# quantum-bitss/Audio-Backdoor-Attack

Hardware: AMD Instinct MI355X
Metric: poisoned+clean utterances/sec/GPU; ASR & clean-acc parity vs reference (higher is better)
Workload: dtype f32 (conv GEMMs as exact 3-way bf16 splits, 6 MFMA terms, fp32 accumulate)

## Files before the change

### audio-backdoor-attack_amd/_lib.py

```python
from __future__ import annotations

import ctypes as C
import os
import threading

HERE = os.path.dirname(os.path.abspath(__file__))
LIB_PATH = os.environ.get("ABD_LIB", os.path.join(HERE, "libabd.so"))

ABD_MEL_HTK, ABD_MEL_SLANEY = 0, 1
ABD_PAD_REFLECT, ABD_PAD_CONSTANT = 0, 1
INJECT_NONE, INJECT_ADD, INJECT_SNR_WINDOW, INJECT_HALF_MIX, INJECT_DEPLOY, INJECT_DEPLOY_CLAMP = 0, 1, 2, 3, 4, 5
MFCC_INFO = {"fast": 0, "ppb": 1, "chunks": 2, "mel_path": 3, "dct_kernel": 4, "bwd_ok": 5}
MFCC_MEL_PATHS = ("generic", "half_slot", "segmented", "blue_slots")
MFCC_DCT_KERNELS = ("plain", "lds", "mfma1", "mfma2", "mfma3")
METRICS_WORDS = 8

EXPORTS = (
    "abd_last_error", "abd_version",
    "abd_mfcc_plan_create", "abd_mfcc_plan_destroy", "abd_mfcc_plan_frames", "abd_mfcc_plan_describe",
    "abd_mfcc_plan_info",
    "abd_mfcc_workspace_bytes", "abd_mfcc_f32", "abd_mfcc_rows_f32", "abd_gather_rows_f32", "abd_inject_waveform_f32", "abd_inject_workspace_bytes",
    "abd_inject_row_scales",
    "abd_pydub_overlay_i16", "abd_mfcc_deploy_backward_workspace_bytes", "abd_mfcc_deploy_backward",
    "abd_smallcnn_create", "abd_smallcnn_destroy", "abd_smallcnn_param_count", "abd_smallcnn_param_offsets",
    "abd_smallcnn_flat_features", "abd_smallcnn_workspace_bytes", "abd_smallcnn_workspace_offset", "abd_smallcnn_bn1_folded", "abd_smallcnn_conv2_planes",
    "abd_smallcnn_train_step",
    "abd_smallcnn_apply", "abd_smallcnn_forward", "abd_smallcnn_backward", "abd_smallcnn_eval", "abd_adam_f32",
    "abd_smallcnn_input_grad_workspace_bytes", "abd_smallcnn_input_grad",
    "abd_smallcnn_ablate_workspace_bytes", "abd_smallcnn_ablate_eval",
    "abd_segment_norms_workspace_bytes", "abd_segment_norms_f32", "abd_perturb_f32", "abd_sgd_f32",
    "abd_smallcnn_finetune_reg_workspace_bytes", "abd_smallcnn_finetune_reg_step",
    "abd_row_abs_sums_f32", "abd_smallcnn_unlearn_workspace_bytes", "abd_smallcnn_unlearn_step",
    "abd_reinit_weights_f32", "abd_smallcnn_unlearn_run", "abd_nwc_pair_f32",
    "abd_smallcnn_hidden_sums", "abd_smallcnn_fcprune_workspace_bytes", "abd_smallcnn_fcprune_eval",
    "abd_smallcnn_pruned_finetune_workspace_bytes", "abd_smallcnn_pruned_finetune_step",
    "abd_lstmattn_create", "abd_lstmattn_destroy", "abd_lstmattn_param_count", "abd_lstmattn_param_offsets",
    "abd_lstmattn_tile_rows", "abd_lstmattn_workspace_bytes", "abd_lstmattn_workspace_offset", "abd_lstmattn_forward",
    "abd_lstmattn_backward", "abd_lstmattn_train_step", "abd_lstmattn_eval",
    "abd_per_utterance_lstmattn_workspace_bytes", "abd_per_utterance_lstmattn_forward",
    "abd_rnn_create", "abd_rnn_destroy", "abd_rnn_param_count", "abd_rnn_param_offsets", "abd_rnn_tile_info",
    "abd_rnn_workspace_bytes", "abd_rnn_workspace_offset", "abd_rnn_forward", "abd_rnn_backward",
    "abd_rnn_train_step", "abd_rnn_eval",
    "abd_largecnn_create", "abd_largecnn_destroy", "abd_largecnn_param_count", "abd_largecnn_param_offsets",
    "abd_largecnn_tile_info", "abd_largecnn_linear_features", "abd_largecnn_workspace_bytes",
    "abd_largecnn_workspace_offset", "abd_largecnn_set_large_min_blocks", "abd_largecnn_forward",
    "abd_largecnn_backward", "abd_largecnn_train_step", "abd_largecnn_eval",
    "abd_resnet_create", "abd_resnet_destroy", "abd_resnet_param_count", "abd_resnet_param_offsets",
    "abd_resnet_running_count", "abd_resnet_running_offsets", "abd_resnet_tile_info", "abd_resnet_linear_features",
    "abd_resnet_workspace_bytes", "abd_resnet_workspace_offset", "abd_resnet_forward", "abd_resnet_backward",
    "abd_resnet_train_step", "abd_resnet_eval",
    "abd_profile_start", "abd_profile_start_every", "abd_profile_step", "abd_profile_stop",
)

PHASES = ("stft_mel", "db_dct", "row_scale", "prep_weights", "conv1_stats", "conv1_bn_pool", "conv2_fwd",
          "bn2_pool", "conv3_fwd", "bn3_pool_dropout", "fc1_fwd", "fc2_loss", "metrics", "fc2_bwd", "fc1_wgrad",
          "fc1_dgrad", "bn3_bwd", "conv3_wgrad", "conv3_dgrad", "bn2_bwd", "conv2_wgrad", "conv2_dgrad",
          "conv1_bwd_wgrad", "adam", "finalize", "head_fwd", "head_mid", "head_bwd", "head_dgrad",
          "feat_gather")
# ... 173 lines not shown
        "abd_mfcc_f32": (i32, [vp, vp, i64, vp, i64, C.POINTER(Inject), vp, vp, sz, vp]),
        "abd_mfcc_rows_f32": (i32, [vp, vp, i64, vp, i64, C.POINTER(Inject), vp, vp, vp, sz, vp]),
        "abd_gather_rows_f32": (i32, [vp, i64, vp, i64, vp, vp]),
        "abd_inject_waveform_f32": (i32, [vp, i64, i64, vp, i64, C.POINTER(Inject), vp, vp, sz, vp]),
        "abd_inject_workspace_bytes": (sz, [i64]),
        "abd_inject_row_scales": (i32, [vp, i64, i64, i64, C.POINTER(Inject), vp, vp]),
        "abd_pydub_overlay_i16": (i32, [vp, i64, vp, i64, vp, i64, vp, vp]),
        "abd_pydub_overlay_ragged_i16": (i32, [vp, i64, vp, vp, i64, i64, vp, i64, i64, vp, vp, vp]),
        "abd_softmax_entropy": (i32, [vp, i64, i32, vp, vp, vp]),
        "abd_style_board_create": (i32, [C.POINTER(Effect), i32, i32, i64, C.POINTER(vp)]),
        "abd_style_board_destroy": (None, [vp]),
        "abd_style_board_apply": (i32, [vp, vp, i64, vp, i64, i64, vp, i64, vp, sz, vp]),
        "abd_style_board_workspace_bytes": (sz, [vp, i64]),
        "abd_resample_plan_create": (i32, [i32, i32, i32, C.c_double, C.POINTER(vp)]),
        "abd_resample_plan_destroy": (None, [vp]),
        "abd_resample_output_length": (i64, [vp, i64]),
        "abd_resample_f32": (i32, [vp, vp, i64, i64, i64, vp, i64, vp]),
        "abd_pair_cross_entropy": (i32, [vp, vp, i64, i32, vp, vp]),
        "abd_smallcnn_forward_per_utterance_workspace_bytes": (sz, [vp, i64]),
        "abd_smallcnn_forward_per_utterance": (i32, [vp, vp, i64, vp, C.c_uint64, C.c_uint64, vp, vp, vp, vp, sz,
                                                     vp]),
        "abd_mfcc_deploy_backward_workspace_bytes": (sz, [vp, i64, i64]),
        "abd_mfcc_deploy_backward": (i32, [vp, vp, i64, vp, i64, C.POINTER(Inject), vp, vp, i32, vp, sz, vp]),
        "abd_smallcnn_create": (i32, [i32, i32, i32, i32, C.POINTER(vp)]),
        "abd_smallcnn_destroy": (None, [vp]),
        "abd_smallcnn_set_precision": (i32, [vp, i32]),
        "abd_smallcnn_param_count": (i64, [vp]),
        "abd_smallcnn_param_offsets": (i32, [vp, C.POINTER(i64)]),
        "abd_smallcnn_flat_features": (i32, [vp]),
        "abd_smallcnn_workspace_bytes": (sz, [vp, i64]),
        "abd_smallcnn_workspace_offset": (i64, [vp, i64, C.c_char_p]),
        "abd_smallcnn_bn1_folded": (C.c_int, [vp, i64]),
        "abd_smallcnn_conv2_planes": (C.c_int, [vp, i64]),
        "abd_smallcnn_train_step": (i32, [vp, C.POINTER(TrainArgs), vp, sz, vp]),
        "abd_smallcnn_apply": (i32, [vp, C.POINTER(TrainArgs), vp, sz, vp]),
        "abd_smallcnn_forward": (i32, [vp, C.POINTER(TrainArgs), i32, vp, sz, vp]),
        "abd_smallcnn_backward": (i32, [vp, C.POINTER(TrainArgs), vp, vp, sz, vp]),
        "abd_smallcnn_eval": (i32, [vp, vp, i64, vp, vp, vp, vp, vp, vp, vp, sz, vp]),
        "abd_adam_f32": (i32, [vp, vp, vp, vp, i64, i64, f32, f32, f32, f32, vp]),
        "abd_smallcnn_input_grad_workspace_bytes": (sz, [vp, i64]),
        "abd_smallcnn_input_grad": (i32, [vp, vp, i64, vp, vp, vp, f32, vp, vp, vp, vp, sz, vp]),
        "abd_smallcnn_ablate_workspace_bytes": (sz, [vp, i64, i32]),
        "abd_smallcnn_ablate_eval": (i32, [vp, vp, i64, vp, vp, vp, vp, i32, i32, i32, vp, vp, vp, sz, vp]),
        "abd_segment_norms_workspace_bytes": (sz, [C.POINTER(i64), i32]),
        "abd_segment_norms_f32": (i32, [vp, C.POINTER(i64), i32, vp, vp, sz, vp]),
        "abd_perturb_f32": (i32, [vp, vp, vp, C.POINTER(i64), i32, f32, vp, vp]),
        "abd_sgd_f32": (i32, [vp, vp, vp, f32, vp, f32, f32, vp, i64, vp]),
        "abd_smallcnn_finetune_reg_workspace_bytes": (sz, [vp, i64]),
        "abd_smallcnn_finetune_reg_step": (i32, [vp, C.POINTER(FinetuneRegArgs), vp, sz, vp]),
        "abd_row_abs_sums_f32": (i32, [vp, vp, C.POINTER(RowSegment), i32, vp, vp, vp]),
        "abd_smallcnn_unlearn_workspace_bytes": (sz, [vp, i64]),
        "abd_smallcnn_unlearn_step": (i32, [vp, C.POINTER(UnlearnArgs), vp, sz, vp]),
        "abd_reinit_weights_f32": (i32, [vp, i64, vp, C.POINTER(RowSegment), i32, vp, C.POINTER(i64), i32, vp, vp, vp,
                                         vp]),
        "abd_smallcnn_unlearn_run": (i32, [vp, C.POINTER(UnlearnArgs), i64, vp, sz, vp]),
        "abd_nwc_pair_f32": (i32, [vp, vp, vp, C.POINTER(RowSegment), i32, vp, vp, vp, vp, vp, vp, vp]),
        "abd_smallcnn_hidden_sums": (i32, [vp, vp, i64, vp, vp, vp, vp, sz, vp]),
        "abd_smallcnn_fcprune_workspace_bytes": (sz, [vp, i64, i32]),
        "abd_smallcnn_fcprune_eval": (i32, [vp, vp, i64, vp, vp, vp, vp, i32, vp, vp, vp, sz, vp]),
        "abd_smallcnn_pruned_finetune_workspace_bytes": (sz, [vp, i64]),
        "abd_smallcnn_pruned_finetune_step": (i32, [vp, C.POINTER(PrunedFinetuneArgs), vp, sz, vp]),
        "abd_lstmattn_create": (i32, [i32, i32, i32, C.POINTER(vp)]),
        "abd_lstmattn_destroy": (None, [vp]),
        "abd_lstmattn_param_count": (i64, [vp]),
        "abd_lstmattn_param_offsets": (i32, [vp, C.POINTER(i64)]),
        "abd_lstmattn_tile_rows": (i32, []),
# ... 118 lines not shown
```

### audio-backdoor-attack_amd/csrc/smallcnn.hip

```cpp
#include "abd_common.h"
#include "prof.h"

#include <algorithm>
#include <type_traits>
#include <cmath>
#include <vector>
#include <map>
#include <array>
#include <mutex>

typedef float f32x16 __attribute__((ext_vector_type(16)));
typedef __bf16 bf16x8 __attribute__((ext_vector_type(8)));
typedef __bf16 bf16x4 __attribute__((ext_vector_type(4)));
typedef __bf16 bf16x2 __attribute__((ext_vector_type(2)));
typedef float f32x2 __attribute__((ext_vector_type(2)));

__device__ __forceinline__ void store_planes4(uint16_t* base, int64_t plane, int64_t e, float4 x, int np) {
  f32x2 v[2] = {f32x2{x.x, x.y}, f32x2{x.z, x.w}};
#pragma unroll
  for (int pl = 0; pl < 3; ++pl) {
    if (pl >= np) break;
    uint32_t u[2];
#pragma unroll
    for (int h = 0; h < 2; ++h) {
// ... 2897 lines not shown
  constexpr int kC1 = 5 * 64;
  if ((int)blockIdx.x < kC1) {
    const int col = blockIdx.x;
    float* g = const_cast<float*>(a.g);
    partial_sum_body(part, nblk, nullptr, g, g + 4 * 64, col);
    if (threadIdx.x == 0) adam_elem(a, col < 4 * 64 ? (col % 64) * 4 + col / 64 : col);
    return;
  }
  const int64_t nb = (int64_t)gridDim.x - kC1;
  for (int64_t i = kC1 + ((int64_t)blockIdx.x - kC1) * kT + threadIdx.x; i < a.n; i += nb * kT) adam_elem(a, i);
}

__global__ void __launch_bounds__(kT) logsoftmax_bwd_kernel(const float* dlp, const float* lp, int B, int K, float* dz) {
  const int lane = threadIdx.x & 63;
  const int row = blockIdx.x * (kT / kWave) + (threadIdx.x >> 6);
  if (row >= B) return;
  const bool act = lane < K;
  const float d = act ? dlp[(int64_t)row * K + lane] : 0.0f;
  const float sd = abd::wave_sum(d);
  if (act) dz[(int64_t)row * K + lane] = d - expf(lp[(int64_t)row * K + lane]) * sd;
}

int grid_for(int64_t total, int cap = 4096) {
  return (int)std::max<int64_t>(1, std::min<int64_t>((total + kT - 1) / kT, cap));
}

}

struct abd_cnn {
  Geo g;
  int max_batch;
  int64_t off[P_COUNT + 1];
  int precision = ABD_PREC_F32_SPLIT;
};

namespace {

struct Work {
  float *p1, *r2, *p2, *r3, *p3d, *d2, *logp, *dz, *rowinfo;
  float *dp3, *da, *dz3, *dp2, *dz2, *dp1;
  float *w2f, *w2d, *w3f, *w3d, *f1t;
  float* part;
  float *partb3, *partb2;
  float* xh3;
  float* hslab;
  float* part3;
  float* daT;
  uint16_t* p1s;
  uint16_t* dz2s;
  unsigned* tickets;
  int ntickets;
  float* w2fold;
  double* ft2;
  float* slab;
  float* slab2;
  float4* coef;
  BCoef* bcoef;
  uint8_t *mask1, *mask2;
  size_t bytes;
};

constexpr int kConv2Slabs = 1024, kConv3Slabs = 1024, kFc1MSplit = 8, kFc1KSplit = 48, kFc2Split = 16;
constexpr int kSlabGroup = 32;

int env_int(const char* name, int dflt) {
  const char* v = getenv(name);
  return v ? atoi(v) : dflt;
}
int c1_rows() { return kR1; }
int64_t nchunks_conv1(const Geo& g, int64_t B) { return B * ((g.H1 + c1_rows() - 1) / c1_rows()); }
int64_t nblk_conv1(const Geo& g, int64_t B) { return std::min<int64_t>(nchunks_conv1(g, B), 2048); }
int64_t c1f_blocks() {
  static int64_t n = 0;
  if (n == 0) {
    int dev = 0, cu = 256, per = 1;
    (void)hipGetDevice(&dev);
    (void)hipDeviceGetAttribute(&cu, hipDeviceAttributeMultiprocessorCount, dev);
    (void)hipOccupancyMaxActiveBlocksPerMultiprocessor(&per, reinterpret_cast<const void*>(&conv1_stats_fold_kernel),
                                                       kT, 0);
    n = (int64_t)cu * std::max(1, per);
  }
  return n;
}
template <bool FULL>
int64_t c1w_blocks() {
  static int64_t n = 0;
  if (n == 0) {
    int dev = 0, cu = 256, per = 1;
    (void)hipGetDevice(&dev);
    (void)hipDeviceGetAttribute(&cu, hipDeviceAttributeMultiprocessorCount, dev);
    (void)hipOccupancyMaxActiveBlocksPerMultiprocessor(&per, reinterpret_cast<const void*>(&conv1_wgrad_kernel<FULL>),
                                                       kT, 0);
    n = (int64_t)cu * std::max(1, per);
  }
  return n;
}
// ... 32 lines not shown
  w.p1 = F(n_p1);
  w.r2 = F(n_r2);
  w.p2 = F(n_p2);
  w.r3 = F(n_r3);
  w.p3d = F(B * g.flat);
  w.d2 = F(B * 128);
  w.logp = F(B * g.K);
  w.dz = F(B * g.K);
  w.rowinfo = F(B * 4);
  w.dp3 = F(B * g.flat);
  w.da = F(B * 128);
  w.dz3 = F(n_r3);
  w.dp2 = F(n_p2);
  w.dz2 = F(n_r2);
  w.dp1 = F(n_p1);
  w.w2f = F(64 * 256);
  w.w2d = F(64 * 256);
  w.w3f = F(32 * 256);
  w.w3d = F(64 * 128);
  w.f1t = F(128LL * g.flat);
  const int64_t pb = std::max<int64_t>({nblk_conv1(g, B) * 64 * 5, 4096LL * 64 * 2,
                                        ((B * g.H2 * g.W2 + kBM - 1) / kBM) * 64 * 2});
  w.part = F(pb);
  const int64_t slab = std::max<int64_t>({(int64_t)kConv2Slabs * 64 * 256, (int64_t)kConv3Slabs * 32 * 256,
                                          (int64_t)kFc1MSplit * 128 * g.flat});
  w.slab = F(slab);
  w.slab2 = F(std::max<int64_t>({(int64_t)(kConv2Slabs / kSlabGroup + 1) * 64 * 256, (int64_t)kFc1KSplit * B * 128,
                                 (int64_t)kFc2Split * 64 * 129}));
  w.coef = reinterpret_cast<float4*>(take(3 * 64 * sizeof(float4)));
  w.bcoef = reinterpret_cast<BCoef*>(take(3 * 64 * sizeof(BCoef)));
  w.mask1 = reinterpret_cast<uint8_t*>(take((size_t)B * g.flat));
  w.mask2 = reinterpret_cast<uint8_t*>(take((size_t)B * 128));
  w.partb3 = F(std::max<int64_t>(4096, head_napply(pool_args(g, 3, B), B)) * 64);
  w.partb2 = F(4096LL * 64);
  w.w2fold = F(64 * 256);
  w.ft2 = reinterpret_cast<double*>(take(64 * 64 * sizeof(double)));
  {
    const HeadPlan hp = head_plan(g, B);
    w.xh3 = F(B * g.flat);
    w.hslab = F((int64_t)hp.ks * B * 128);
    w.part3 = F((int64_t)hp.nrb * hp.nft * 64);
    w.daT = F(128 * B);
  }
  w.p1s = reinterpret_cast<uint16_t*>(take((size_t)3 * n_p1 * sizeof(uint16_t)));
  w.dz2s = reinterpret_cast<uint16_t*>(take((size_t)3 * n_r2 * sizeof(uint16_t)));
  w.ntickets = kGuardTickets;
  w.tickets = reinterpret_cast<unsigned*>(take((size_t)w.ntickets * sizeof(unsigned)));
  w.bytes = off;
  return w;
}

struct Params {
  const float* p[P_COUNT];
};

Params params_of(const abd_cnn* net, const float* flat) {
  Params r;
  for (int i = 0; i < P_COUNT; ++i) r.p[i] = flat + net->off[i];
  return r;
}

PrepArgs prep_args(const Params& P, const Work& w, const Geo& g) {
  return PrepArgs{P.p[P_C2W], P.p[P_C3W], P.p[P_F1W], g.flat, w.w2f, w.w2d, w.w3f, w.w3d, w.f1t, w.tickets, w.ntickets};
}
unsigned prep_blocks(const Geo& g) { return (unsigned)grid_for(64 * 256 + 32 * 256 + 128LL * g.flat); }

PoolArgs pool_args(const Geo& g, int layer, int64_t B) {
// ... 300 lines not shown
    per_cu = std::max(1, per_cu);
    cached_lds = lds;
  }
  int grid = (int)std::min<int64_t>({(int64_t)a.nchunks, (int64_t)n_cu * per_cu, (int64_t)max_slabs});
  a.per = (a.nchunks + grid - 1) / grid;
  grid = (a.nchunks + a.per - 1) / a.per;
  if (phase >= 0) abd::prof_begin(phase, s);
  kern<<<grid, kT, lds, s>>>(a);
  if (phase >= 0) abd::prof_end(phase, s);
  ABD_LAUNCH_CHECK();
  return grid;
}


int ws_grid() {
  static int n = 0;
  if (n == 0) {
    int dev = 0, cu = 256;
    (void)hipGetDevice(&dev);
    (void)hipDeviceGetAttribute(&cu, hipDeviceAttributeMultiprocessorCount, dev);
    n = std::max(1, cu);
  }
  return n;
}
int ws_blocks(int64_t M, int rows_per_block = 8 * 32) {
  const int64_t need = (M + rows_per_block - 1) / rows_per_block;
  return (int)std::max<int64_t>(1, std::min<int64_t>(ws_grid(), need));
}
bool ws_fits(const NTArgs& a) {
  return a.taps == 4 && a.ksplit <= 1 && a.ldb == 4 * a.Cs && a.ldc == a.N &&
         (int64_t)a.Hs * a.Ws * a.Cs * 4 * (a.M / (a.Ho * a.Wo)) < 0x7ffffff0LL;
}
int ws_dma_mode() { return env_int("ABD_WS_DMA", 1); }
int dma_span(const NTArgs& a) {
  static std::mutex mu;
  static std::map<std::array<int, 12>, int> cache;
  const std::array<int, 12> key{a.Hs, a.Ws, a.Ho, a.Wo, a.dh[0], a.dh[1], a.dh[2], a.dh[3], a.dw[0], a.dw[1], a.dw[2], a.dw[3]};
  std::lock_guard<std::mutex> lk(mu);
  auto it = cache.find(key);
  if (it != cache.end()) return it->second;
  const int HoWo = a.Ho * a.Wo, n = 2 * HoWo + 32;
  int tmin = 0, tmax = 0;
  for (int t = 0; t < 4; ++t) {
    tmin = std::min(tmin, a.dh[t] * a.Ws + a.dw[t]);
    tmax = std::max(tmax, a.dh[t] * a.Ws + a.dw[t]);
  }
  auto src = [&](int m) {
    const int b = m / HoWo, rem = m % HoWo, h = rem / a.Wo, w = rem % a.Wo;
    return (b * a.Hs + h) * a.Ws + w;
  };
  int span = 0;
  for (int m0 = 0; m0 + 32 <= n; ++m0) {
    int lo = INT32_MAX, hi = INT32_MIN;
    for (int r = 0; r < 32; ++r) {
      lo = std::min(lo, src(m0 + r));
      hi = std::max(hi, src(m0 + r));
    }
    span = std::max(span, hi + tmax - (lo + tmin) + 1);
  }
  cache[key] = span;
  return span;
}
enum WsKind { WS_SPEC, WS_DMA, WS_SPLIT };
template <int EPI, int NP, bool PA>
WsKind ws_kind(const NTArgs& a) {
  static_assert(!PA || NP == 1, "plane operands: bf16's single plane");
// ... 341 lines not shown
    ABD_LAUNCH_CHECK();
  }
  return 0;
}

bool bn1_fold_ok(const abd_cnn* net, const Geo& g, int64_t B) {
  return (net->precision == ABD_PREC_F32_SPLIT || net->precision == ABD_PREC_BF16) &&
         (int64_t)g.H1 * g.W1p * 64 * 4 * B < 0x7ffffff0LL;
}
int conv2_planes(const abd_cnn* net, const Geo& g, int64_t B, bool fold1) {
  if (!fold1) return 0;
  const int np = net->precision == ABD_PREC_BF16 ? 1 : 0;
  if (np == 0) return 0;
  const int64_t n_p1 = B * g.H1 * g.W1p * 64, n_r2 = B * g.H2 * g.W2 * 64;
  if ((int64_t)3 * std::max(n_p1, n_r2) * 2 >= 0x7ffffff0LL) return 0;
  if (!trp_planes_fit<2>(g.H2, g.W2, g.H1, g.W1p)) return 0;
  return np;
}

constexpr int kGuardBlocks = 64;
int bn_bwd_guard(const PoolArgs& pa_in, const float* gamma, const float* beta, double count, const float4* coef,
                 float* dgamma, float* dbeta, BCoef* bcoef, unsigned* ticket, hipStream_t s) {
  PoolArgs pa = pa_in;
  pa.nblk = std::min(grid_for((int64_t)pa.B * pa.Ho * pa.Wo * pa.C / 4), kGuardBlocks);
  bn_pool_bwd_stats_guard_kernel<<<pa.nblk, kT, 0, s>>>(
      PoolGuard{pa, gamma, beta, GuardOut{count, coef, dgamma, dbeta, bcoef, ticket}});
  ABD_LAUNCH_CHECK();
  return 0;
}

int backward(abd_cnn* net, const Work& w, const Params& P, float* grads, const float* x, int64_t B,
             const DropArgs& drop1, hipStream_t s, void* fc_grads_event, const BnSync& sy = BnSync{},
             int64_t* metrics = nullptr, bool fold1 = false, double loss_w = 1.0, const HeadArgs* head = nullptr,
             int planes = 0, int* c1_defer = nullptr) {
  const bool derive = !sy.on();
  int bn3_parts = 0;
  const Geo& g = net->g;
  float* G[P_COUNT];
  for (int i = 0; i < P_COUNT; ++i) G[i] = grads + net->off[i];
  const float s2 = 1.0f / (1.0f - kP2);
  if (head) {
    if (launch_head(3, *head, s)) return -1;
    if (fc_grads_event) ABD_HIP(hipEventRecord(static_cast<hipEvent_t>(fc_grads_event), s));
  } else {
  abd::prof_begin(abd::PH_FC2_BWD, s);
  {
    const int rows = (int)((B + kFc2Split - 1) / kFc2Split);
    const int nw = (g.K * kFc2Split + 1) / 2;
    fc2_grads_kernel<<<(unsigned)(nw + grid_for(B * 128) + (metrics ? 1 : 0)), kT, 0, s>>>(
        w.dz, w.d2, P.p[P_F2W], (int)B, g.K, rows, kFc2Split, w.slab2, s2, w.da, nw, w.rowinfo, metrics, loss_w);
    fc2_reduce_colsum_kernel<<<(unsigned)(128 + (g.K * 129 + kT - 1) / kT), kT, 0, s>>>(
        w.slab2, kFc2Split, g.K, G[P_F2W], G[P_F2B], w.da, (int)B, 128, G[P_F1B]);
  }
  abd::prof_end(abd::PH_FC2_BWD, s);
  ABD_LAUNCH_CHECK();
  {
    TNArgs a{};
    a.D = w.da;
    a.ldd = 128;
    a.src = w.p3d;
    a.Hs = a.Ws = a.Ho = a.Wo = 1;
    a.Cs = g.flat;
    a.M = (int)B;
    a.taps = 1;
    a.N = 128;
    a.Ktot = g.flat;
    a.mchunk = (int)((B + kFc1MSplit - 1) / kFc1MSplit);
// ... 87 lines not shown
      return -1;
    const DeriveArgs dv2{nullptr, P.p[P_C3W], G[P_C3B], P.p[P_BN2W], P.p[P_BN2B], w.coef + 64, (double)B * g.H2 * g.W2,
                         G[P_BN2W], G[P_BN2B], w.bcoef + 64};
    PoolArgs pg = pool_args(g, 2, B);
    pg.r = w.r2;
    pg.coef = w.coef + 64;
    pg.dp = w.dp2;
    pg.part = w.part;
    pg.nblk = 64;
    const PoolGuard guard2{pg, P.p[P_BN2W], P.p[P_BN2B],
                           GuardOut{(double)B * g.H2 * g.W2, w.coef + 64, G[P_BN2W], G[P_BN2B], w.bcoef + 64,
                                    w.tickets + 1}};
    if (nsl < 0 || (derive ? reduce_slabs(w, nsl, 32, 256, 64, G[P_C3W], s, BiasSum{w.partb3, pa.nblk, 32, G[P_C3B]},
                                          &dv2, nullptr, guard2)
                           : reduce_slabs(w, nsl, 32, 256, 64, G[P_C3W], s, BiasSum{w.partb3, pa.nblk, 32, G[P_C3B]})))
      return -1;
  }
  int nsl2 = -1, pa_nblk2 = 0;
  {
    PoolArgs pa = pool_args(g, 2, B);
    pa.r = w.r2;
    pa.coef = w.coef + 64;
    pa.dp = w.dp2;
    pa.part = w.part;
    pa.nblk = grid_for(B * pa.Ho * pa.Wo * 64 / 4);
    if (!derive) {
      bn_pool_bwd_stats_kernel<<<pa.nblk, kT, 0, s>>>(pa);
      ABD_LAUNCH_CHECK();
      if (bn_bwd_finalize(sy, 4, w.part, pa.nblk, 64, (double)B * g.H2 * g.W2, P.p[P_BN2W], w.coef + 64, G[P_BN2W],
                          G[P_BN2B], w.bcoef + 64, s))
        return -1;
    }
    pa.bcoef = w.bcoef + 64;
    pa.dz = w.dz2;
    if (planes > 0) {
      pa.dzs = w.dz2s;
      pa.dzplane = B * g.H2 * g.W2 * 64;
      pa.dznp = planes;
    }
    pa.part = w.partb2;
    pa.nblk = grid_for(B * win_ext_h(pa) * win_ext_w(pa) * 64 / 4);
    abd::prof_begin(abd::PH_BN2_BWD, s);
    bn_bwd_apply_kernel<<<pa.nblk, kT, 0, s>>>(pa, win_ext_h(pa), win_ext_w(pa));
    abd::prof_end(abd::PH_BN2_BWD, s);
    ABD_LAUNCH_CHECK();
    pa_nblk2 = pa.nblk;
    const WgPlanes wpl{w.dz2s, w.p1s, B * g.H2 * g.W2 * 64, B * g.H1 * g.W1p * 64};
    int nsl = planes == 1 ? launch_wgrad_tr_planes<2, 1>(g.H2, g.W2, g.H1, g.W1p, B, kConv2Slabs, w.slab,
                                                         abd::PH_CONV2_WGRAD, s, wpl)
              : net->precision == ABD_PREC_BF16
                  ? launch_wgrad_tr<2, 64, 1>(w.dz2, w.p1, g.H2, g.W2, g.H1, g.W1p, B, kConv2Slabs, w.slab,
                                              abd::PH_CONV2_WGRAD, s)
              : net->precision == ABD_PREC_F32_SPLIT
                  ? launch_wgrad_tr<2, 64>(w.dz2, w.p1, g.H2, g.W2, g.H1, g.W1p, B, kConv2Slabs, w.slab,
                                           abd::PH_CONV2_WGRAD, s)
                  : -1;
    ABD_CHECK(planes == 0 || nsl >= 0, ABD_E_UNSUPPORTED, "conv2 plane-mode weight gradient geometry");
    if (nsl < 0)
      nsl = launch_wgrad_rows<64, 64>(w.dz2, w.p1, g.H2, g.W2, g.H1, g.W1p, B, 1, kConv2Slabs, w.slab,
                                      abd::PH_CONV2_WGRAD, s);
    nsl2 = nsl;
    NTArgs da = conv_dgrad_args(w.dz2, g.H2, g.W2, 64, g.H1, g.W1p, B, w.w2d, 64, w.dp1);
    if (planes > 0) {
      da.srcs = w.dz2s;
      da.splane = B * g.H2 * g.W2 * 64;
    }
    const bool ws2 = net->precision != ABD_PREC_F32 && ws_fits(da);
    if ((planes == 1 ? launch_conv_ws_split<EPI_STORE, 1, true>(da, s, abd::PH_CONV2_DGRAD)
         : ws2 ? (net->precision == ABD_PREC_BF16 ? launch_conv_ws_split<EPI_STORE, 1>(da, s, abd::PH_CONV2_DGRAD)
                                                  : launch_conv_ws_split<EPI_STORE>(da, s, abd::PH_CONV2_DGRAD))
               : launch_nt<64, EPI_STORE>(da, s, abd::PH_CONV2_DGRAD)))
      return -1;
  }
  {
    C1Args c1{};
    c1.x = x;
    c1.w = P.p[P_C1W];
    c1.b = P.p[P_C1B];
    c1.coef = w.coef;
    c1.dp1 = w.dp1;
    c1.part = w.part;
    c1.g = g;
    c1.B = (int)B;
    c1.nblk = (int)nblk_conv1(g, B);
    c1.rows = c1_rows();
    const DeriveArgs dv1{fold1 ? w.coef : nullptr, P.p[P_C2W], G[P_C2B], P.p[P_BN1W], P.p[P_BN1B], w.coef, (double)B * g.H1 * g.W1,
                         G[P_BN1W], G[P_BN1B], w.bcoef};
    if (derive) {
      C1Args c1g = c1;
      c1g.nblk = 64;
      const C1Guard guard1{c1g, P.p[P_BN1W], P.p[P_BN1B],
                           GuardOut{(double)B * g.H1 * g.W1, w.coef, G[P_BN1W], G[P_BN1B], w.bcoef, w.tickets + 0}};
      if (nsl2 < 0 || reduce_slabs(w, nsl2, 64, 256, 64, G[P_C2W], s, BiasSum{w.partb2, pa_nblk2, 64, G[P_C2B]}, &dv1,
                                  fold1 ? w.coef : nullptr, guard1))
        return -1;
    } else {
      if (nsl2 < 0 || reduce_slabs(w, nsl2, 64, 256, 64, G[P_C2W], s, BiasSum{w.partb2, pa_nblk2, 64, G[P_C2B]}, nullptr,
                                  fold1 ? w.coef : nullptr))
        return -1;
      conv1_bwd_stats_kernel<<<c1.nblk, kT, 0, s>>>(c1);
      ABD_LAUNCH_CHECK();
      if (bn_bwd_finalize(sy, 5, w.part, c1.nblk, 64, (double)B * g.H1 * g.W1, P.p[P_BN1W], w.coef, G[P_BN1W],
                          G[P_BN1B], w.bcoef, s))
        return -1;
    }
// ... 35 lines not shown
}

}

extern "C" {

int abd_smallcnn_create(int H0, int W0, int num_classes, int max_batch, abd_cnn** net) {
  ABD_CHECK(net != nullptr, ABD_E_INVALID, "NULL out pointer");
  ABD_CHECK(num_classes >= 1 && num_classes <= 64, ABD_E_UNSUPPORTED, "num_classes must be in [1, 64]");
  Geo g = make_geo(H0, W0, num_classes);
  ABD_CHECK(H0 >= 8 && W0 >= 8 && W0 <= 128 && g.W3 >= 1 && g.H3 >= 2, ABD_E_UNSUPPORTED,
            "input %dx%d too small/large for smallcnn", H0, W0);
  ABD_CHECK(g.flat % 32 == 0, ABD_E_UNSUPPORTED, "flat features %d not a multiple of 32", g.flat);
  auto* n = new abd_cnn();
  n->g = g;
  n->max_batch = max_batch;
  int64_t sz[P_COUNT];
  param_sizes(g, sz);
  n->off[0] = 0;
  for (int i = 0; i < P_COUNT; ++i) n->off[i + 1] = n->off[i] + sz[i];
  *net = n;
  return ABD_OK;
}

void abd_smallcnn_destroy(abd_cnn* net) { delete net; }

int abd_smallcnn_set_precision(abd_cnn* net, int precision) {
  ABD_CHECK(net != nullptr, ABD_E_INVALID, "NULL net");
  ABD_CHECK(precision == ABD_PREC_F32 || precision == ABD_PREC_BF16 || precision == ABD_PREC_F32_SPLIT, ABD_E_INVALID, "unknown precision %d", precision);
  net->precision = precision;
  return ABD_OK;
}

int64_t abd_smallcnn_param_count(const abd_cnn* net) { return net ? net->off[P_COUNT] : -1; }

int abd_smallcnn_param_offsets(const abd_cnn* net, int64_t* offsets) {
  ABD_CHECK(net && offsets, ABD_E_INVALID, "NULL argument");
  for (int i = 0; i <= P_COUNT; ++i) offsets[i] = net->off[i];
  return ABD_OK;
}

int abd_smallcnn_flat_features(const abd_cnn* net) { return net ? net->g.flat : -1; }

size_t abd_smallcnn_workspace_bytes(const abd_cnn* net, int64_t batch) {
  if (!net) return 0;
  return layout(net, batch, nullptr).bytes;
}

int abd_smallcnn_bn1_folded(const abd_cnn* net, int64_t batch) {
  return (net && batch >= 1 && bn1_fold_ok(net, net->g, batch)) ? 1 : 0;
}

int abd_smallcnn_conv2_planes(const abd_cnn* net, int64_t batch) {
  if (!net || batch < 1) return 0;
  return conv2_planes(net, net->g, batch, bn1_fold_ok(net, net->g, batch));
}

int64_t abd_smallcnn_workspace_offset(const abd_cnn* net, int64_t batch, const char* name) {
  if (!net || !name) return -1;
  char* base = reinterpret_cast<char*>(static_cast<uintptr_t>(4096));
  const Work w = layout(net, batch, base);
  const struct {
    const char* n;
    const void* p;
  } tab[] = {{"p1", w.p1},     {"r2", w.r2},       {"p2", w.p2},     {"r3", w.r3},       {"p3d", w.p3d},
             {"d2", w.d2},     {"logp", w.logp},   {"dz", w.dz},     {"dp3", w.dp3},     {"da", w.da},
// ... 11 lines not shown
  const int64_t B = a->batch;
  ABD_CHECK(B >= 1, ABD_E_INVALID, "train step needs batch >= 1, got %lld", (long long)B);
  ABD_CHECK(B * net->g.H1 * net->g.W1p * 64 < (1LL << 31), ABD_E_INVALID, "batch too large (int32 activation offsets)");
  const Work w = layout(net, B, static_cast<char*>(workspace));
  ABD_CHECK(workspace && workspace_bytes >= w.bytes, ABD_E_WORKSPACE, "workspace too small (%zu < %zu)",
            workspace_bytes, w.bytes);
  ABD_CHECK(!a->do_update || (a->exp_avg && a->exp_avg_sq && a->adam_step >= 1), ABD_E_INVALID, "Adam state missing");
  hipStream_t s = static_cast<hipStream_t>(stream);
  const Geo& g = net->g;
  Params P = params_of(net, a->params);
  const PrepArgs prep = prep_args(P, w, g);
  const bool fold1 = bn1_fold_ok(net, g, B) && !bn_sync_of(a).on();
  DropArgs d1 = make_drop(a, 1, w.mask1, g.flat), d2 = make_drop(a, 2, w.mask2, 128);
  const BnSync sy = bn_sync_of(a);
  const float inv = (a->grad_scale > 0.0f ? a->grad_scale : 1.0f) / (float)B;
  const double loss_w = a->grad_scale > 0.0f ? (double)a->grad_scale : 1.0;
  const bool use_head = head_on() && !sy.on();
  HeadArgs ha{};
  if (use_head)
    ha = head_args(net, w, P, a->grads, B, d1, d2, a->labels, a->indicators, inv, a->logprobs_out, a->metrics, loss_w);
  const int planes = conv2_planes(net, g, B, fold1);
  if (forward(net, w, P, a->x, B, a->running, a->running, true, d1, d2, s, a->num_batches_tracked, nullptr, sy, &prep,
              fold1, use_head ? &ha : nullptr, planes))
    return -1;
  if (use_head) {
    if (launch_head(2, ha, s)) return -1;
  } else {
    if (loss_and_metrics(net, w, P, a->labels, a->indicators, B, inv, true, a->logprobs_out, nullptr, s)) return -1;
  }
  const bool defer = a->do_update && !sy.on() && net->off[P_C1W] == 0 && net->off[P_C1B] == 4 * 64 &&
                     net->off[P_BN1W] == 5 * 64;
  int c1_nblk = 0;
  if (backward(net, w, P, a->grads, a->x, B, d1, s, a->fc_grads_event, sy, a->metrics, fold1, loss_w,
               use_head ? &ha : nullptr, planes, defer ? &c1_nblk : nullptr))
    return -1;
  copy_masks(a, w, g, B, s);
  if (defer) {
    const double bc1 = 1.0 - pow((double)a->beta1, (double)a->adam_step);
    const double bc2 = 1.0 - pow((double)a->beta2, (double)a->adam_step);
    const int64_t n = net->off[P_COUNT];
    const AdamArgs aa{a->params, a->grads, a->exp_avg, a->exp_avg_sq, n, (float)(1.0 - (double)a->beta1), a->beta2,
                      (float)(1.0 - (double)a->beta2), (float)((double)a->lr / bc1), (float)sqrt(bc2), a->eps};
    abd::prof_begin(abd::PH_ADAM, s);
    adam_c1_kernel<<<5 * 64 + (unsigned)grid_for(n - 5 * 64, 2048), kT, 0, s>>>(aa, w.part, c1_nblk);
    abd::prof_end(abd::PH_ADAM, s);
    ABD_LAUNCH_CHECK();
  } else if (a->do_update) {
    int rc = abd_smallcnn_apply(net, a, workspace, workspace_bytes, stream);
    if (rc) return rc;
  }
  return ABD_OK;
}

int abd_smallcnn_forward(abd_cnn* net, const abd_train_args* a, int train_mode, void* workspace,
                         size_t workspace_bytes, abd_stream_t stream) {
  ABD_CHECK(net && a && a->x && a->params && a->running && a->logprobs_out, ABD_E_INVALID, "NULL argument");
  const int64_t B = a->batch;
  ABD_CHECK(B >= 1, ABD_E_INVALID, "bad batch %lld", (long long)B);
  ABD_CHECK(B * net->g.H1 * net->g.W1p * 64 < (1LL << 31), ABD_E_INVALID, "batch too large (int32 activation offsets)");
  const Work w = layout(net, B, static_cast<char*>(workspace));
  ABD_CHECK(workspace && workspace_bytes >= w.bytes, ABD_E_WORKSPACE, "workspace too small (%zu < %zu)",
            workspace_bytes, w.bytes);
  hipStream_t s = static_cast<hipStream_t>(stream);
  const Geo& g = net->g;
  Params P = params_of(net, a->params);
  prep_weights_kernel<<<prep_blocks(g), kT, 0, s>>>(prep_args(P, w, g));
  ABD_LAUNCH_CHECK();
// ... 200 lines not shown
```

### include/abd.h

```cpp
#ifndef ABD_H_
#define ABD_H_

#include <stddef.h>
#include <stdint.h>

#ifdef __cplusplus
extern "C" {
#endif

typedef void* abd_stream_t;

#define ABD_OK 0
#define ABD_E_INVALID 1001
#define ABD_E_UNSUPPORTED 1002
#define ABD_E_WORKSPACE 1003

const char* abd_last_error(void);
int abd_version(void);

enum { ABD_MEL_HTK = 0, ABD_MEL_SLANEY = 1 };
enum { ABD_PAD_REFLECT = 0, ABD_PAD_CONSTANT = 1 };

typedef struct abd_mfcc_plan abd_mfcc_plan;

// ... 80 lines not shown
int64_t abd_resample_output_length(const abd_resample_plan* plan, int64_t length);
int abd_resample_f32(const abd_resample_plan* plan, const float* in, int64_t in_stride, int64_t batch,
                     int64_t length, float* out, int64_t out_stride, abd_stream_t stream);

enum { ABD_FX_GAIN = 0, ABD_FX_DISTORTION = 1, ABD_FX_LADDER = 2, ABD_FX_PHASER = 3, ABD_FX_CHORUS = 4,
       ABD_FX_REVERB = 5, ABD_FX_PITCHSHIFT = 6 };
typedef struct abd_effect {
  int kind;
  float p[8];
} abd_effect;
typedef struct abd_style_board abd_style_board;
int abd_style_board_create(const abd_effect* fx, int n, int sample_rate, int64_t max_length,
                           abd_style_board** board);
void abd_style_board_destroy(abd_style_board* board);
size_t abd_style_board_workspace_bytes(const abd_style_board* board, int64_t batch);
int abd_style_board_apply(const abd_style_board* board, const float* in, int64_t in_stride,
                          const int32_t* rows, int64_t batch, int64_t length, float* out,
                          int64_t out_stride, void* workspace, size_t workspace_bytes,
                          abd_stream_t stream);

typedef struct abd_cnn abd_cnn;

int abd_smallcnn_create(int H0, int W0, int num_classes, int max_batch, abd_cnn** net);
enum { ABD_PREC_F32 = 0, ABD_PREC_BF16 = 1, ABD_PREC_F32_SPLIT = 2 };
int abd_smallcnn_set_precision(abd_cnn* net, int precision);
void abd_smallcnn_destroy(abd_cnn* net);
int64_t abd_smallcnn_param_count(const abd_cnn* net);
int abd_smallcnn_param_offsets(const abd_cnn* net, int64_t* offsets );
int abd_smallcnn_flat_features(const abd_cnn* net);
size_t abd_smallcnn_workspace_bytes(const abd_cnn* net, int64_t batch);
int64_t abd_smallcnn_workspace_offset(const abd_cnn* net, int64_t batch, const char* name);
int abd_smallcnn_bn1_folded(const abd_cnn* net, int64_t batch);
int abd_smallcnn_conv2_planes(const abd_cnn* net, int64_t batch);

#define ABD_METRICS_WORDS 8

typedef struct abd_train_args {
  const float* x;
  const int64_t* labels;
  const int64_t* indicators;
  int64_t batch;
  float* params;
  float* grads;
  float* exp_avg;
  float* exp_avg_sq;
  float* running;
  int64_t adam_step;
  float lr, beta1, beta2, eps;
  int do_update;
  const uint8_t* mask1_in;
  const uint8_t* mask2_in;
  uint64_t seed, counter;
  uint8_t* mask1_out;
  uint8_t* mask2_out;
  float* logprobs_out;
  int64_t* metrics;
  float grad_scale;
  int64_t* num_batches_tracked;
  void* fc_grads_event;
  int64_t row_offset;
  double* bn_sync_buf;
  int (*bn_sync)(void* ctx, int point, int64_t offset, int64_t n);
  void* bn_sync_ctx;
} abd_train_args;
#define ABD_BN_SYNC_STRIDE 136

// ... 346 lines not shown
```

Measured before the change: 660,000.

## Split conv2 backward into batch chunks with configurable chunk count

Restructures the conv2 backward stage (BN2 backward apply, weight-gradient slabs, data-gradient conv) into a loop over batch chunks. Each chunk writes its own partial-sum and slab ranges, and the partb2 buffer grows to hold up to four chunks. The chunk count is set through a new API or the ABD_BWD_CHUNKS environment variable and defaults to 1, so the default behaviour keeps the single-chunk schedule apart from the small index and setup changes. The aim is to keep each chunk's working set resident in cache, at the cost of more kernel launches.

```diff
diff --git a/audio-backdoor-attack_amd/_lib.py b/audio-backdoor-attack_amd/_lib.py
--- a/audio-backdoor-attack_amd/_lib.py
+++ b/audio-backdoor-attack_amd/_lib.py
@@ -24,6 +24,7 @@
     "abd_pydub_overlay_i16", "abd_mfcc_deploy_backward_workspace_bytes", "abd_mfcc_deploy_backward",
     "abd_smallcnn_create", "abd_smallcnn_destroy", "abd_smallcnn_param_count", "abd_smallcnn_param_offsets",
     "abd_smallcnn_flat_features", "abd_smallcnn_workspace_bytes", "abd_smallcnn_workspace_offset", "abd_smallcnn_bn1_folded", "abd_smallcnn_conv2_planes",
+    "abd_smallcnn_set_bwd_chunks", "abd_smallcnn_bwd_chunks",
     "abd_smallcnn_train_step",
     "abd_smallcnn_apply", "abd_smallcnn_forward", "abd_smallcnn_backward", "abd_smallcnn_eval", "abd_adam_f32",
     "abd_smallcnn_input_grad_workspace_bytes", "abd_smallcnn_input_grad",
@@ -263,6 +264,8 @@
         "abd_smallcnn_workspace_offset": (i64, [vp, i64, C.c_char_p]),
         "abd_smallcnn_bn1_folded": (C.c_int, [vp, i64]),
         "abd_smallcnn_conv2_planes": (C.c_int, [vp, i64]),
+        "abd_smallcnn_set_bwd_chunks": (i32, [vp, i32]),
+        "abd_smallcnn_bwd_chunks": (C.c_int, [vp]),
         "abd_smallcnn_train_step": (i32, [vp, C.POINTER(TrainArgs), vp, sz, vp]),
         "abd_smallcnn_apply": (i32, [vp, C.POINTER(TrainArgs), vp, sz, vp]),
         "abd_smallcnn_forward": (i32, [vp, C.POINTER(TrainArgs), i32, vp, sz, vp]),
diff --git a/audio-backdoor-attack_amd/csrc/smallcnn.hip b/audio-backdoor-attack_amd/csrc/smallcnn.hip
--- a/audio-backdoor-attack_amd/csrc/smallcnn.hip
+++ b/audio-backdoor-attack_amd/csrc/smallcnn.hip
@@ -2953,6 +2953,7 @@
   int max_batch;
   int64_t off[P_COUNT + 1];
   int precision = ABD_PREC_F32_SPLIT;
+  int bwd_chunks = 0;
 };
 
 namespace {
@@ -2983,6 +2984,7 @@
 
 constexpr int kConv2Slabs = 1024, kConv3Slabs = 1024, kFc1MSplit = 8, kFc1KSplit = 48, kFc2Split = 16;
 constexpr int kSlabGroup = 32;
+constexpr int kMaxBwdChunks = 4, kBwdChunksDefault = 1;
 
 int env_int(const char* name, int dflt) {
   const char* v = getenv(name);
@@ -3081,7 +3083,7 @@
   w.mask1 = reinterpret_cast<uint8_t*>(take((size_t)B * g.flat));
   w.mask2 = reinterpret_cast<uint8_t*>(take((size_t)B * 128));
   w.partb3 = F(std::max<int64_t>(4096, head_napply(pool_args(g, 3, B), B)) * 64);
-  w.partb2 = F(4096LL * 64);
+  w.partb2 = F(4096LL * 64 * kMaxBwdChunks);
   w.w2fold = F(64 * 256);
   w.ft2 = reinterpret_cast<double*>(take(64 * 64 * sizeof(double)));
   {
@@ -3448,6 +3450,10 @@
          (int64_t)a.Hs * a.Ws * a.Cs * 4 * (a.M / (a.Ho * a.Wo)) < 0x7ffffff0LL;
 }
 int ws_dma_mode() { return env_int("ABD_WS_DMA", 1); }
+int bwd_chunks_default() {
+  static const int n = std::min(std::max(env_int("ABD_BWD_CHUNKS", kBwdChunksDefault), 1), kMaxBwdChunks);
+  return n;
+}
 int dma_span(const NTArgs& a) {
   static std::mutex mu;
   static std::map<std::array<int, 12>, int> cache;
@@ -3855,7 +3861,7 @@
 int backward(abd_cnn* net, const Work& w, const Params& P, float* grads, const float* x, int64_t B,
              const DropArgs& drop1, hipStream_t s, void* fc_grads_event, const BnSync& sy = BnSync{},
              int64_t* metrics = nullptr, bool fold1 = false, double loss_w = 1.0, const HeadArgs* head = nullptr,
-             int planes = 0, int* c1_defer = nullptr) {
+             int planes = 0, int* c1_defer = nullptr, int chunks = 1) {
   const bool derive = !sy.on();
   int bn3_parts = 0;
   const Geo& g = net->g;
@@ -4009,45 +4015,65 @@
         return -1;
     }
     pa.bcoef = w.bcoef + 64;
-    pa.dz = w.dz2;
-    if (planes > 0) {
-      pa.dzs = w.dz2s;
-      pa.dzplane = B * g.H2 * g.W2 * 64;
-      pa.dznp = planes;
-    }
-    pa.part = w.partb2;
-    pa.nblk = grid_for(B * win_ext_h(pa) * win_ext_w(pa) * 64 / 4);
-    abd::prof_begin(abd::PH_BN2_BWD, s);
-    bn_bwd_apply_kernel<<<pa.nblk, kT, 0, s>>>(pa, win_ext_h(pa), win_ext_w(pa));
-    abd::prof_end(abd::PH_BN2_BWD, s);
-    ABD_LAUNCH_CHECK();
-    pa_nblk2 = pa.nblk;
-    const WgPlanes wpl{w.dz2s, w.p1s, B * g.H2 * g.W2 * 64, B * g.H1 * g.W1p * 64};
-    int nsl = planes == 1 ? launch_wgrad_tr_planes<2, 1>(g.H2, g.W2, g.H1, g.W1p, B, kConv2Slabs, w.slab,
-                                                         abd::PH_CONV2_WGRAD, s, wpl)
-              : net->precision == ABD_PREC_BF16
-                  ? launch_wgrad_tr<2, 64, 1>(w.dz2, w.p1, g.H2, g.W2, g.H1, g.W1p, B, kConv2Slabs, w.slab,
-                                              abd::PH_CONV2_WGRAD, s)
-              : net->precision == ABD_PREC_F32_SPLIT
-                  ? launch_wgrad_tr<2, 64>(w.dz2, w.p1, g.H2, g.W2, g.H1, g.W1p, B, kConv2Slabs, w.slab,
-                                           abd::PH_CONV2_WGRAD, s)
-                  : -1;
-    ABD_CHECK(planes == 0 || nsl >= 0, ABD_E_UNSUPPORTED, "conv2 plane-mode weight gradient geometry");
-    if (nsl < 0)
-      nsl = launch_wgrad_rows<64, 64>(w.dz2, w.p1, g.H2, g.W2, g.H1, g.W1p, B, 1, kConv2Slabs, w.slab,
-                                      abd::PH_CONV2_WGRAD, s);
-    nsl2 = nsl;
-    NTArgs da = conv_dgrad_args(w.dz2, g.H2, g.W2, 64, g.H1, g.W1p, B, w.w2d, 64, w.dp1);
-    if (planes > 0) {
-      da.srcs = w.dz2s;
-      da.splane = B * g.H2 * g.W2 * 64;
-    }
-    const bool ws2 = net->precision != ABD_PREC_F32 && ws_fits(da);
-    if ((planes == 1 ? launch_conv_ws_split<EPI_STORE, 1, true>(da, s, abd::PH_CONV2_DGRAD)
-         : ws2 ? (net->precision == ABD_PREC_BF16 ? launch_conv_ws_split<EPI_STORE, 1>(da, s, abd::PH_CONV2_DGRAD)
-                                                  : launch_conv_ws_split<EPI_STORE>(da, s, abd::PH_CONV2_DGRAD))
-               : launch_nt<64, EPI_STORE>(da, s, abd::PH_CONV2_DGRAD)))
-      return -1;
+    const int nch = (int)std::min<int64_t>(std::max(1, chunks), kMaxBwdChunks);
+    const int64_t Bc = (B + nch - 1) / nch;
+    const int64_t e_r2 = (int64_t)g.H2 * g.W2 * 64, e_p2 = (int64_t)g.H2p * g.W2p * 64, e_p1 = (int64_t)g.H1 * g.W1p * 64;
+    const int64_t wext = (int64_t)win_ext_h(pa) * win_ext_w(pa) * 64 / 4;
+    for (int64_t b0 = 0; b0 < B; b0 += Bc) pa_nblk2 += grid_for(std::min(Bc, B - b0) * wext);
+    int blk0 = 0;
+    nsl2 = 0;
+    for (int64_t b0 = 0; b0 < B; b0 += Bc) {
+      const int64_t bc = std::min(Bc, B - b0);
+      PoolArgs pc = pa;
+      pc.B = (int)bc;
+      pc.r = w.r2 + b0 * e_r2;
+      pc.dp = w.dp2 + b0 * e_p2;
+      pc.dz = w.dz2 + b0 * e_r2;
+      if (planes > 0) {
+        pc.dzs = w.dz2s + b0 * e_r2;
+        pc.dzplane = B * e_r2;
+        pc.dznp = planes;
+      }
+      pc.part = w.partb2 + blk0;
+      pc.nblk = pa_nblk2;
+      const int nb = grid_for(bc * wext);
+      blk0 += nb;
+      abd::prof_begin(abd::PH_BN2_BWD, s);
+      bn_bwd_apply_kernel<<<nb, kT, 0, s>>>(pc, win_ext_h(pc), win_ext_w(pc));
+      abd::prof_end(abd::PH_BN2_BWD, s);
+      ABD_LAUNCH_CHECK();
+      const float* dz2c = w.dz2 + b0 * e_r2;
+      const float* p1c = w.p1 + b0 * e_p1;
+      float* slabc = w.slab + (int64_t)nsl2 * 64 * 256;
+      const int max_slabs = kConv2Slabs / nch;
+      const WgPlanes wpl{w.dz2s + b0 * e_r2, w.p1s + b0 * e_p1, B * e_r2, B * e_p1};
+      int nsl = planes == 1 ? launch_wgrad_tr_planes<2, 1>(g.H2, g.W2, g.H1, g.W1p, bc, max_slabs, slabc,
+                                                           abd::PH_CONV2_WGRAD, s, wpl)
+                : net->precision == ABD_PREC_BF16
+                    ? launch_wgrad_tr<2, 64, 1>(dz2c, p1c, g.H2, g.W2, g.H1, g.W1p, bc, max_slabs, slabc,
+                                                abd::PH_CONV2_WGRAD, s)
+                : net->precision == ABD_PREC_F32_SPLIT
+                    ? launch_wgrad_tr<2, 64>(dz2c, p1c, g.H2, g.W2, g.H1, g.W1p, bc, max_slabs, slabc,
+                                             abd::PH_CONV2_WGRAD, s)
+                    : -1;
+      ABD_CHECK(planes == 0 || nsl >= 0, ABD_E_UNSUPPORTED, "conv2 plane-mode weight gradient geometry");
+      if (nsl < 0)
+        nsl = launch_wgrad_rows<64, 64>(dz2c, p1c, g.H2, g.W2, g.H1, g.W1p, bc, 1, max_slabs, slabc,
+                                        abd::PH_CONV2_WGRAD, s);
+      if (nsl < 0) return -1;
+      nsl2 += nsl;
+      NTArgs da = conv_dgrad_args(dz2c, g.H2, g.W2, 64, g.H1, g.W1p, bc, w.w2d, 64, w.dp1 + b0 * e_p1);
+      if (planes > 0) {
+        da.srcs = w.dz2s + b0 * e_r2;
+        da.splane = planes == 1 ? bc * e_r2 : B * e_r2;
+      }
+      const bool ws2 = net->precision != ABD_PREC_F32 && ws_fits(da);
+      if ((planes == 1 ? launch_conv_ws_split<EPI_STORE, 1, true>(da, s, abd::PH_CONV2_DGRAD)
+           : ws2 ? (net->precision == ABD_PREC_BF16 ? launch_conv_ws_split<EPI_STORE, 1>(da, s, abd::PH_CONV2_DGRAD)
+                                                    : launch_conv_ws_split<EPI_STORE>(da, s, abd::PH_CONV2_DGRAD))
+                 : launch_nt<64, EPI_STORE>(da, s, abd::PH_CONV2_DGRAD)))
+        return -1;
+    }
   }
   {
     C1Args c1{};
@@ -4149,6 +4175,18 @@
   return ABD_OK;
 }
 
+int abd_smallcnn_set_bwd_chunks(abd_cnn* net, int chunks) {
+  ABD_CHECK(net != nullptr, ABD_E_INVALID, "NULL net");
+  ABD_CHECK(chunks >= 0 && chunks <= kMaxBwdChunks, ABD_E_INVALID, "bwd chunks %d not in [0, %d]", chunks, kMaxBwdChunks);
+  net->bwd_chunks = chunks;
+  return ABD_OK;
+}
+
+int abd_smallcnn_bwd_chunks(const abd_cnn* net) {
+  if (!net) return -1;
+  return net->bwd_chunks > 0 ? net->bwd_chunks : bwd_chunks_default();
+}
+
 int64_t abd_smallcnn_param_count(const abd_cnn* net) { return net ? net->off[P_COUNT] : -1; }
 
 int abd_smallcnn_param_offsets(const abd_cnn* net, int64_t* offsets) {
@@ -4226,7 +4264,8 @@
                      net->off[P_BN1W] == 5 * 64;
   int c1_nblk = 0;
   if (backward(net, w, P, a->grads, a->x, B, d1, s, a->fc_grads_event, sy, a->metrics, fold1, loss_w,
-               use_head ? &ha : nullptr, planes, defer ? &c1_nblk : nullptr))
+               use_head ? &ha : nullptr, planes, defer ? &c1_nblk : nullptr,
+               net->bwd_chunks > 0 ? net->bwd_chunks : bwd_chunks_default()))
     return -1;
   copy_masks(a, w, g, B, s);
   if (defer) {
diff --git a/include/abd.h b/include/abd.h
--- a/include/abd.h
+++ b/include/abd.h
@@ -136,6 +136,8 @@
 int64_t abd_smallcnn_workspace_offset(const abd_cnn* net, int64_t batch, const char* name);
 int abd_smallcnn_bn1_folded(const abd_cnn* net, int64_t batch);
 int abd_smallcnn_conv2_planes(const abd_cnn* net, int64_t batch);
+int abd_smallcnn_set_bwd_chunks(abd_cnn* net, int chunks);
+int abd_smallcnn_bwd_chunks(const abd_cnn* net);
 
 #define ABD_METRICS_WORDS 8
 
```

After: 659,000. No clear change (-0.1%).
